# yeyupiaoling/PPASR

Hardware: AMD Instinct MI355X
Metric: audio-seconds/s (RTF^-1) Conformer-streaming fbank, batch32 per GPU, ctc_greedy (higher is better)
Workload: dtype f32

## Files before the change

### ppasr_amd/csrc/capi.hip

```cpp
#include <cxxabi.h>
#include <cstdlib>

#include "capi_internal.h"

namespace ppasr {
thread_local LaunchProf g_launch_prof;
}

static thread_local std::string g_err;
std::string& ppasr_err_slot() { return g_err; }


ppasr_status upload_pe_table(ppasr_model_s* m, BlobMap& sd, const float** pe_dev) {
  const int d = m->desc.output_size > 0 ? m->desc.output_size : kD;
  const int max_len = m->desc.max_len > 0 ? m->desc.max_len : 5000;
  m->desc.max_len = max_len;
  std::vector<float> pe((size_t)max_len * d);
  auto it = sd.find("__pe_table__");
  if (it != sd.end() && it->second.numel() == pe.size()) {
    std::memcpy(pe.data(), it->second.p, pe.size() * sizeof(float));
  } else {
    for (int i = 0; i < d / 2; ++i) {
      float div = expf((float)(2 * i) * (float)(-(std::log(10000.0) / d)));
      for (int pos = 0; pos < max_len; ++pos) {
// ... 152 lines not shown
    GET(istd, "encoder.global_cmvn.istd", F);
    GET(ew, "encoder.embed.out.0.weight", (size_t)F * d);
    GET(eb, "encoder.embed.out.0.bias", d);
    GET(lg, "encoder.embed.out.1.weight", d);
    GET(lb, "encoder.embed.out.1.bias", d);
    UP(vec_of(mean, F), m->front.cmvn_mean);
    UP(vec_of(istd, F), m->front.cmvn_istd);
    m->lin_kpad = (F + 255) / 256 * 256;
    UP4(pack_b(m->lin_kpad, d, [&](int k, int n) { return k < F ? ew[(size_t)k * d + n] : 0.f; }), m->front.embed_w);
    UP(vec_of(eb, d), m->front.embed_b);
    UP(vec_of(lg, d), m->lin_ln_g);
    UP(vec_of(lb, d), m->lin_ln_b);
    m->front.conv1_w = m->front.conv1_b = m->front.conv2_b = nullptr;
    m->front.conv2_w = nullptr;
  } else {
    GET(mean, "encoder.global_cmvn.mean", F);
    GET(istd, "encoder.global_cmvn.istd", F);
    GET(c1w, "encoder.embed.conv.0.weight", d * 9);
    GET(c1b, "encoder.embed.conv.0.bias", d);
    const int k2 = il == 6 ? 5 : 3;
    GET(c2w, "encoder.embed.conv.2.weight", (size_t)d * d * k2 * k2);
    GET(c2b, "encoder.embed.conv.2.bias", d);
    const std::string lin = il ? "encoder.embed.linear" : "encoder.embed.out.0";
    GET(ew, lin + ".weight", (size_t)d * F2 * d);
    GET(eb, lin + ".bias", d);
    UP(vec_of(mean, F), m->front.cmvn_mean);
    UP(vec_of(istd, F), m->front.cmvn_istd);
    std::vector<float> c1(9 * d);
    for (int c = 0; c < d; ++c)
      for (int j = 0; j < 9; ++j) c1[j * d + c] = c1w[c * 9 + j];
    UP(c1, m->front.conv1_w);
    UP(vec_of(c1b, d), m->front.conv1_b);
    const int taps2 = k2 * k2;
    UP4(pack_b(taps2 * d, d, [&](int k, int n) { return c2w[((size_t)n * d + (k % d)) * taps2 + (k / d)]; }), m->front.conv2_w);
    UP(vec_of(c2b, d), m->front.conv2_b);
    m->front.conv2_k = k2;
    m->front.conv2_s = il == 6 ? 3 : 2;
    m->front.conv3_w = nullptr;
    m->front.conv3_b = nullptr;
    if (il == 8) {
      GET(c3w, "encoder.embed.conv.4.weight", (size_t)d * d * 9);
      GET(c3b, "encoder.embed.conv.4.bias", d);
      UP4(pack_b(9 * d, d, [&](int k, int n) { return c3w[((size_t)n * d + (k % d)) * 9 + (k / d)]; }), m->front.conv3_w);
      UP(vec_of(c3b, d), m->front.conv3_b);
    }
    UP4(pack_b(F2 * d, d, [&](int k, int n) { return ew[((size_t)(k % d) * F2 + (k / d)) * d + n]; }), m->front.embed_w);
    UP(vec_of(eb, d), m->front.embed_b);
  }

  const float* pe_dev = nullptr;
  if ((st = upload_pe_table(m, sd, &pe_dev)) != PPASR_OK) return st;
  m->pe_dev = pe_dev;
  UP(std::vector<float>(d, 0.f), m->zero_vec);
  if (generic) m->gen_x.resize(desc->num_blocks);
  const int max_len = m->desc.max_len;
  m->layers.resize(desc->num_blocks);
  m->layer_ks.assign(desc->num_blocks, KS);
  m->layer_group.assign(desc->num_blocks, 1);
  for (int i = 0; i < desc->num_blocks; ++i) {
    LayerW& L = m->layers[i];
    const int KSi = eff ? (KS >> eff_strides_before(*desc, i)) : KS;
    const bool grouped = eff && ((desc->group_layer_mask >> i) & 1);
    m->layer_ks[i] = KSi;
    m->layer_group[i] = grouped ? desc->group_size : 1;
    const int pbn = grouped ? desc->group_size * d : d;
    const std::string p = "encoder.encoders." + std::to_string(i) + ".";
    auto ln = [&](const std::string& n, const float** g, const float** b) -> ppasr_status {
// ... 511 lines not shown
    };
    fn();
    g_launch_prof = LaunchProf{};
  };
  const bool eff = h->desc.model_type == PPASR_MODEL_EFFICIENT_CONFORMER;
  const bool skip = h->skip_padding && lens && !h->taps && h->desc.input_layer != 1;
  const bool skip_front = skip && h->desc.input_layer == 0;
  const int rc = h->desc.causal ? 0 : (h->desc.cnn_module_kernel - 1) / 2;
  const int slack_half = rc + 4, slack_full = eff ? 2 * slack_half + rc + 8 : rc + 4;
  auto pskip = [&](int Tcur, int mul_cur) {
    PadSkip ps;
    if (skip) {
      ps.lens = lens;
      ps.Tp = Tcur;
      ps.mul = mul_cur;
      ps.slack = mul_cur == sub ? slack_full : slack_half;
    }
    return ps;
  };
  const f32x4* conv2_h3 = h->gemm_mode == PPASR_GEMM_F16X3 ? h->conv2_w_h3 : nullptr;
  const bool conv12 = h->desc.input_layer == 0 && !conv2_h3 && conv12_enabled(h) && conv12_supported(h->front, F, F2);
  const PadSkip ps_front = skip_front ? pskip(Tp, sub) : PadSkip{};
  if (!conv12) timed(0, [&] { launch_conv1(feats, h->front, y1, B, T, F, T1, F1, st, ps_front); });
  if (h->desc.input_layer == 8) {
    timed(1, [&] {
      launch_conv_stage(y1, h->front.conv2_w, h->front.conv2_b, y2, B, T1, F1, fd.T2, F2, 3, 2, st);
      launch_conv_stage(y2, h->front.conv3_w, h->front.conv3_b, y1, B, fd.T2, F2, Tp, h->F3, 3, 2, st);
    });
    timed(2, [&] { launch_embed(y1, h->front, xa, M, h->F3 * kD, sqrtf((float)kD), false, st, PadSkip{}, ffn_split_for(h, M), y2); });
  } else {
    timed(1, [&] {
      int* tile_tab = (size_t)B + 2 <= ((size_t)M + 63) / 64 * 64 ? reinterpret_cast<int*>(ws + wl.rmax) : nullptr;
      if (conv12) launch_conv12(feats, h->front, y2, B, T, F, Tp, F2, st, ps_front, tile_tab);
      else launch_conv2(y1, h->front, y2, B, T1, F1, Tp, F2, st, ps_front, tile_tab, h->desc.input_layer == 0 ? conv2_h3 : nullptr);
    });
    timed(2, [&] {
      launch_embed(y2, h->front, xa, M, F2 * kD, sqrtf((float)kD), false, st, ps_front, wide_slices_for(h, M, F2), y1,
                   conv2_h3 ? h->embed_w_h3 : nullptr);
    });
  }
  tap(xa, (size_t)M * kD);
  const int n_chunks = h->desc.linear_units / 256;
  struct BlkTab { int Ti, R; int* tab; } btabs[4];
  int n_bt = 0;
  size_t bt_off = ((size_t)B + 2 + 15) / 16 * 16;
  const bool bt_ok = skip && block_tables_enabled() && (size_t)B + 2 <= ((size_t)M + 63) / 64 * 64;
  auto with_table = [&](PadSkip p, int Tcur, int R) {
    if (!bt_ok) return p;
    for (int k = 0; k < n_bt; ++k)
      if (btabs[k].Ti == Tcur && btabs[k].R == R) { p.tab = btabs[k].tab; return p; }
    const size_t n = 1 + ((size_t)B * Tcur + R - 1) / R;
    if (n_bt == 4 || bt_off + n > 2 * (((size_t)M + 63) / 64 * 64)) return p;
    int* t = reinterpret_cast<int*>(ws + wl.rmax) + bt_off;
    launch_block_table(p, B * Tcur, R, t, st);
    btabs[n_bt++] = BlkTab{Tcur, R, t};
    bt_off += (n + 15) / 16 * 16;
    p.tab = t;
    return p;
  };
  int Ti = Tp, mul = sub, pstride = 1;
  bool s1_done = false;
  for (int i = 0; i < h->desc.num_blocks; ++i) {
    const LayerW& L = h->layers[i];
    const int Mi = B * Ti;
    const int grp = h->layer_group[i];
    constexpr int fuse_min_blocks = 128;
// ... 757 lines not shown
```

### ppasr_amd/csrc/capi_internal.h

```cpp
#pragma once
#include <hip/hip_runtime.h>

#include <cmath>
#include <cstdio>
#include <cstring>
#include <memory>
#include <string>
#include <unordered_map>
#include <vector>

#include "../../include/ppasr_hip.h"
#include "conformer_kernels.h"
#include "launch.h"
#include "ctc_beam.h"

using namespace ppasr;

#include "squeezeformer_kernels.h"
#include "ds2_kernels.h"

std::string& ppasr_err_slot();
inline ppasr_status fail(ppasr_status s, const std::string& msg) {
  ppasr_err_slot() = msg;
  return s;
}
#define HIP_TRY(expr)                                                                              \
  do {                                                                                             \
    hipError_t _e = (expr);                                                                        \
    if (_e != hipSuccess) return fail(PPASR_EHIP, std::string(#expr) + ": " + hipGetErrorString(_e)); \
  } while (0)

struct Blob {
  const float* p;
  int ndim;
  int64_t shape[4];
  size_t numel() const {
    size_t n = 1;
    for (int i = 0; i < ndim; ++i) n *= (size_t)shape[i];
    return n;
  }
};

template <typename Acc>
inline std::vector<float> pack_b(int K, int N, Acc w) {
  const int n_tiles = (N + 31) / 32, G = K / 8;
  std::vector<float> out((size_t)n_tiles * G * 256, 0.f);
  for (int nt = 0; nt < n_tiles; ++nt)
    for (int g = 0; g < G; ++g)
      for (int l = 0; l < 64; ++l) {
        int n = nt * 32 + (l & 31);
        if (n >= N) continue;
        float* dst = &out[(((size_t)nt * G + g) * 64 + l) * 4];
        for (int j = 0; j < 4; ++j) dst[j] = w(8 * g + 4 * (l >> 5) + j, n);
      }
  return out;
}

typedef std::unordered_map<std::string, Blob> BlobMap;

inline unsigned eff_stride_mask(const ppasr_model_desc& d) {
  if (d.model_type != PPASR_MODEL_EFFICIENT_CONFORMER) return 0u;
  if (d.stride_layer_mask != 0) return (unsigned)d.stride_layer_mask;
  return d.stride_layer_idx >= 0 ? (1u << d.stride_layer_idx) : 0u;
}
inline int eff_strides_before(const ppasr_model_desc& d, int layer) {
  return __builtin_popcount(eff_stride_mask(d) & ((1u << layer) - 1u));
}

struct ppasr_model_s {
  ppasr_model_desc desc;
  int F1, F2;
  const f32x4* gen_head_w = nullptr;
  const float* gen_head_b = nullptr;
  int gen_vpad = 0;
  int F3 = 0;
  struct Front {
    int T1, T2, Tp;
  };
  int sub_rate() const { return desc.input_layer == 1 ? 1 : desc.input_layer ? desc.input_layer : 4; }
  int F_last() const { return desc.input_layer == 8 ? F3 : F2; }
  int min_frames() const { return desc.input_layer == 1 ? 1 : desc.input_layer == 6 ? 11 : desc.input_layer == 8 ? 15 : 7; }
  Front front_dims(int T) const {
    if (desc.input_layer == 1) return Front{0, 0, T};
    Front f{(T - 1) / 2, 0, 0};
    if (desc.input_layer == 6) {
      f.Tp = (f.T1 - 5) / 3 + 1;
    } else if (desc.input_layer == 8) {
      f.T2 = (f.T1 - 1) / 2;
// ... 151 lines not shown
```

### ppasr_amd/csrc/capi_squeezeformer.hip

```cpp
#include "capi_internal.h"

namespace {

struct Getter {
  BlobMap& sd;
  std::string missing;
  const float* operator()(const std::string& name, size_t numel) {
    auto it = sd.find(name);
    if (it == sd.end() || it->second.numel() != numel) {
      if (missing.empty()) missing = name;
      return nullptr;
    }
    return it->second.p;
  }
};

std::vector<float> vec_of(const float* p, size_t n) { return std::vector<float>(p, p + n); }

}

#define GETW(var, name, numel)                 \
  const float* var = get(name, (size_t)(numel)); \
  if (!var) return fail(PPASR_EMISSING, "missing or mis-shaped weight: " + get.missing)
#define UP(vec, dst) \
// ... 11 lines not shown
  ppasr_status st;
  const bool no_ada = (dsc.options & PPASR_OPT_SQ_NO_ADAPTIVE_SCALE) != 0;
  const std::vector<float> ones_d(d, 1.f), zeros_d(d, 0.f);
  auto adapt = [&](const float*& as, const float*& ab) {
    if (no_ada) {
      as = ones_d.data();
      ab = zeros_d.data();
    }
  };
  {
    GETW(mean, "encoder.global_cmvn.mean", F);
    GETW(istd, "encoder.global_cmvn.istd", F);
    GETW(c1w, "encoder.embed.pw_conv.weight", d * 9);
    GETW(c1b, "encoder.embed.pw_conv.bias", d);
    const float* c2w = get("encoder.embed.dw_conv.weight", (size_t)d * d * 9);
    const bool dw_stride = !c2w;
    if (!c2w) {
      get.missing.clear();
      c2w = get("encoder.embed.dw_conv.weight", (size_t)d * 9);
    }
    if (!c2w) return fail(PPASR_EMISSING, "missing or mis-shaped weight: " + get.missing);
    GETW(c2b, "encoder.embed.dw_conv.bias", d);
    GETW(ew, "encoder.embed.input_proj.0.weight", (size_t)d * F2 * d);
    GETW(eb, "encoder.embed.input_proj.0.bias", d);
    GETW(pg, "encoder.preln.weight", d);
    GETW(pb, "encoder.preln.bias", d);
    UP(vec_of(mean, F), m->front.cmvn_mean);
    UP(vec_of(istd, F), m->front.cmvn_istd);
    std::vector<float> c1(9 * d);
    for (int c = 0; c < d; ++c)
      for (int j = 0; j < 9; ++j) c1[j * d + c] = c1w[c * 9 + j];
    UP(c1, m->front.conv1_w);
    UP(vec_of(c1b, d), m->front.conv1_b);
    UP4(pack_b(9 * d, d, [&](int k, int n) {
          if (dw_stride) return (k % d) == n ? c2w[(size_t)n * 9 + (k / d)] : 0.f;
          return c2w[((size_t)n * d + (k % d)) * 9 + (k / d)];
        }), m->front.conv2_w);
    UP(vec_of(c2b, d), m->front.conv2_b);
    UP4(pack_b(F2 * d, d, [&](int k, int n) { return ew[((size_t)(k % d) * F2 + (k / d)) * d + n]; }), m->front.embed_w);
    UP(vec_of(eb, d), m->front.embed_b);
    UP(vec_of(pg, d), m->preln_g);
    UP(vec_of(pb, d), m->preln_b);
  }
  m->sq_layers.resize(L);
  for (int i = 0; i < L; ++i) {
    SqLayerW& W = m->sq_layers[i];
    const std::string p = "encoder.encoders." + std::to_string(i) + ".";
    auto ln = [&](const std::string& n, const float** g, const float** b) -> ppasr_status {
      const float* gw = get(p + n + ".weight", d);
      const float* gb = get(p + n + ".bias", d);
      if (!gw || !gb) return fail(PPASR_EMISSING, "missing or mis-shaped weight: " + get.missing);
      ppasr_status s1 = m->upload(vec_of(gw, d), g);
      return s1 != PPASR_OK ? s1 : m->upload(vec_of(gb, d), b);
    };
    if ((st = ln("layer_norm1", &W.ln1_g, &W.ln1_b)) != PPASR_OK) return st;
    if ((st = ln("layer_norm2", &W.ln2_g, &W.ln2_b)) != PPASR_OK) return st;
    if ((st = ln("layer_norm3", &W.ln3_g, &W.ln3_b)) != PPASR_OK) return st;
    if ((st = ln("layer_norm4", &W.ln4_g, &W.ln4_b)) != PPASR_OK) return st;
    W.cm_eps = 1e-5f;
    if (sd.find(p + "conv_module.norm._mean") != sd.end()) {
      const float* mean = get(p + "conv_module.norm._mean", d);
      const float* var = get(p + "conv_module.norm._variance", d);
      const float* gw = get(p + "conv_module.norm.weight", d);
      const float* gb = get(p + "conv_module.norm.bias", d);
      if (!mean || !var || !gw || !gb) return fail(PPASR_EMISSING, "missing or mis-shaped weight: " + get.missing);
      std::vector<float> sc(d), sh(d);
      for (int c = 0; c < d; ++c) {
        sc[c] = gw[c] / std::sqrt(var[c] + 1e-5f);
        sh[c] = gb[c] - mean[c] * sc[c];
      }
// ... 220 lines not shown
  const int rc = causal ? 0 : (KS - 1) / 2;
  auto pskip = [&](int Tcur, int mul_cur) {
    PadSkip ps;
    if (skip) {
      ps.lens = lens;
      ps.Tp = Tcur;
      ps.mul = mul_cur;
      ps.slack = mul_cur == 4 ? 2 * (rc + 4) + rc + 8 : rc + 4;
    }
    return ps;
  };
  const PadSkip psF = pskip(Tp, 4), psH = pskip(Tr, 8);
  int* tile_tab = (size_t)B + 2 <= ((size_t)M + 63) / 64 * 64 ? reinterpret_cast<int*>(ws + wl.rmax) : nullptr;
  const int rowsF = h->taps ? 32 : row_block_for(h, B, Tp, 4, psF.slack, skip);
  const int rowsH = h->taps ? 32 : row_block_for(h, B, Tr, 8, psH.slack, skip);
  PadSkip psF_rb = psF, psH_rb = psH;
  if (skip && tile_tab && block_tables_enabled()) {
    const int RF = rowsF == 16 ? 16 : 32, RH = rowsH == 16 ? 16 : 32;
    const size_t nF = 1 + ((size_t)M + RF - 1) / RF, nH = 1 + ((size_t)B * Tr + RH - 1) / RH;
    const size_t o1 = ((size_t)B + 2 + 15) / 16 * 16, o2 = o1 + (nF + 15) / 16 * 16;
    if (o2 + nH <= 2 * (((size_t)M + 63) / 64 * 64)) {
      int* base = reinterpret_cast<int*>(ws + wl.rmax);
      launch_block_table(psF, M, RF, base + o1, st);
      launch_block_table(psH, B * Tr, RH, base + o2, st);
      psF_rb.tab = base + o1;
      psH_rb.tab = base + o2;
    }
  }
  const f32x4* conv2_h3 = h->gemm_mode == PPASR_GEMM_F16X3 ? h->conv2_w_h3 : nullptr;
  if (!conv2_h3 && conv12_enabled(h) && conv12_supported(h->front, F, F2)) {
    launch_conv12(feats, h->front, y2, B, T, F, Tp, F2, st, psF, tile_tab);
  } else {
    launch_conv1(feats, h->front, y1, B, T, F, T1, F1, st, psF);
    launch_conv2(y1, h->front, y2, B, T1, F1, Tp, F2, st, psF, tile_tab, conv2_h3);
  }
  launch_embed(y2, h->front, xa, M, F2 * kD, sqrtf((float)kD), true, st,
               (rowsF != 16 && ffn_split_for(h, M) == 1) ? psF_rb : psF, ffn_split_for(h, M), y1,
               conv2_h3 ? h->embed_w_h3 : nullptr);
  launch_ln_rows(xa, h->preln_g, h->preln_b, M, st, psF);
  tap(xa, (size_t)M * kD);
  float* x = xa;
  float* other = xb;
  bool reduced = false;
  bool have_qkv = false;
  for (int i = 0; i < L; ++i) {
    const SqLayerW& W = h->sq_layers[i];
    if (i == h->desc.reduce_idx) {
      HIP_TRY(hipMemcpyAsync(xs, x, (size_t)M * kD * sizeof(float), hipMemcpyDeviceToDevice, st));
      launch_sq_reduce(x, other, qkv, h->sq_reduce, W.wqkv, W.bqkv, lens, B, Tp, Tr, st, psH);
      std::swap(x, other);
      reduced = true;
      have_qkv = true;
    }
    if (i == h->desc.recover_idx && reduced) {
      launch_sq_recover(x, xs, other, qkv, h->sq_wrec, h->sq_brec, W.wqkv, W.bqkv, B, Tp, Tr, st, psF);
      std::swap(x, other);
      reduced = false;
      have_qkv = true;
    }
    const int Ti = reduced ? Tr : Tp;
    const int Mi = B * Ti;
    const int mul = reduced ? 8 : 4;
    const PadSkip& ps = reduced ? psH : psF;
    const bool views16 = ffn_split_for(h, Mi) > 1 && !(rowsF == 16 && h->ffn_split < 0) && Mi <= kSplitRows16Max &&
                         !(h->gemm_mode == PPASR_GEMM_F16X3 && !h->sq_layers_h3.empty());
    auto qkv_view = [](const SqLayerW& w) {
      LayerW v{};
// ... 76 lines not shown
```

### ppasr_amd/csrc/conformer_kernels.h

```cpp
#pragma once
#include <hip/hip_runtime.h>
#include <stdint.h>

#include "rowblock.h"

namespace ppasr {

struct LayerW {
  const float *ln_mac_g, *ln_mac_b, *ln_mha_g, *ln_mha_b, *ln_conv_g, *ln_conv_b;
  const float *ln_ff_g, *ln_ff_b, *ln_fin_g, *ln_fin_b, *ln_cm_g, *ln_cm_b;
  float cm_eps;
  const f32x4 *ffm_w1, *ffm_w2, *ff_w1, *ff_w2, *wqkv, *wo, *pw1, *pw2;
  const float *ffm_b1, *ffm_b2, *ff_b1, *ff_b2, *bqkv, *bo, *pw1_b, *pw2_b;
  const float *dw_w;
  const float *dw_b;
  const float *glu_pad;
  const float *pos_u, *pos_v;
  const float *ptab;
};

struct FrontW {
  const float *cmvn_mean, *cmvn_istd;
  const float *conv1_w, *conv1_b;
  const f32x4 *conv2_w;
  const float *conv2_b;
  int conv2_k = 3, conv2_s = 2;
  const f32x4 *conv3_w = nullptr;
  const float *conv3_b = nullptr;
  const f32x4 *embed_w;
  const float *embed_b;
};

struct HeadW {
  const float *ln_g, *ln_b;
  const f32x4 *w;
  const float *b;
  int V, n_tiles;
};

struct SessDesc {
  int sess;
  int cache_t;
  int pos0;
  int pad;
};

struct AttnArgs {
  const float* q;
  int q_stride;
  const float* k;
  int k_stride;
  const float* v;
  int v_stride;
  int T1, T2;
  int pos0;
  const int64_t* lens;
  float* ctx;
  const float *pos_u, *pos_v;
  const float* ptab;
  int pos_stride;
  int mask_mul;
  int q_frames, kv_frames;
  int group;
  const SessDesc* sess;
  long long sess_stride;
  int pad_skip;
  const float* vt = nullptr;
  int vt_stride = 0;
  int dm = 256;
};
struct VtOut {
  float* vt = nullptr;
  int stride = 0;
  int k_h3 = 0;
};

constexpr size_t kLdsExclusive = 82 * 1024;
size_t ragged_lds(size_t lds, const PadSkip& ps, int n_blocks);

bool launch_attention_t(const AttnArgs& a, int B, int H, hipStream_t st);
hipError_t configure_attention_kernels();

void launch_block_table(const PadSkip& ps, int M, int R, int* tab, hipStream_t st);

bool conv12_supported(const FrontW& fw, int F, int F2);
void launch_conv12(const float* feats, const FrontW& fw, float* y2, int B, int T, int F, int Tp, int F2, hipStream_t st,
                   const PadSkip& ps_frames, int* tile_scratch);
hipError_t configure_front_fused_kernels();

void launch_ffn_qkv_16(const float* x_in, float* x1, float* qkv, const LayerW& w, int M, int n_chunks, hipStream_t st,
                       const PadSkip& ps);
void launch_out_glu_16(const float* ctx, const float* x1, float* x2, float* g, const LayerW& w, const int64_t* lens, int M,
                       int Tp, int mask_mul, hipStream_t st, const PadSkip& ps);
void launch_out_glu_split_16(const float* ctx, const float* x1, float* x2, float* g, float* xhat, const LayerW& w,
                             const int64_t* lens, int M, int Tp, int mask_mul, hipStream_t st, const PadSkip& ps,
                             float* hist = nullptr, int lo = 0);
void launch_shift_caches(float* kc, float* vc, long long layer_stride, int D, int n_layers, int from_full, int keep_full,
                         int from_half, int keep_half, unsigned long long half_mask, hipStream_t st);
void launch_oproj_ln_16(const float* ctx, const float* x1, float* x2_sink, float* xhat_out, const LayerW& w, int M,
                        hipStream_t st, const PadSkip& ps = PadSkip{});
void launch_pw1_glu_cols_16(const float* x, float* g, const LayerW& w, int M, hipStream_t st, float* hist = nullptr, int lo = 0,
                            const float* hist_scale = nullptr, const float* hist_bias = nullptr, const PadSkip& ps = PadSkip{},
                            const int64_t* lens = nullptr, int Tp = 1, int mask_mul = 1);
bool conv_ffn_16_supported(int ksize, int Tp);
void launch_conv_ffn_16(const float* g, const float* x2, float* x_out, const LayerW& w, const int64_t* lens, int M, int Tp,
                        int n_chunks, int ksize, int mask_mul, const LayerW* next, float* x1_next, float* qkv_next,
                        hipStream_t st, bool causal, const PadSkip& ps);
void launch_ffn_qkv_w16(const float* x_in, float* x1, float* qkv, const LayerW& w, int M, int n_chunks, hipStream_t st,
                        const PadSkip& ps, VtOut vt);
void launch_out_glu_w16(const float* ctx, const float* x1, float* x2, float* g, const LayerW& w, const int64_t* lens, int M,
                        int Tp, int mask_mul, hipStream_t st, const PadSkip& ps);
void launch_conv_ffn_w16(const float* g, const float* x2, float* x_out, const LayerW& w, const int64_t* lens, int M, int Tp,
                         int n_chunks, int ksize, int mask_mul, const LayerW* next, float* x1_next, float* qkv_next,
                         hipStream_t st, bool causal, const PadSkip& ps, VtOut vt_next);
hipError_t configure_conformer_t_kernels();

void launch_posproj(const float* pe, const float* wpos , const float* bpos_or_null, float* ptab,
                    int max_len, hipStream_t st, int d = 256);
void launch_conv1(const float* feats, const FrontW& fw, float* y1, int B, int T, int F, int T1, int F1, hipStream_t st,
                  const PadSkip& ps = PadSkip{}, int channels = 256);
// ... 107 lines not shown
```

### ppasr_amd/csrc/front_fused.hip

```cpp
#include "conformer_kernels.h"
#include "launch.h"

namespace ppasr {

template <int MT>
__global__ __launch_bounds__(kThreads) void k_conv12(const float* __restrict__ feats, FrontW fw, float* __restrict__ out,
                                                     int T, int F, int Tp, int F2, int M, int m0, PadSkip ps,
                                                     const int* __restrict__ tile_tab) {
  constexpr int BM = 32 * MT, KC = 128, LD = KC + 4, G = KC / 8, NL = 2 * MT, STEP = G / NL, N_CHUNKS = 18;
  int r0 = m0 + blockIdx.x * BM, Mlim = M;
  if (tile_tab) {
    const int t = blockIdx.x, nb = tile_tab[0];
    const int* pre = tile_tab + 1;
    if (t >= pre[nb]) return;
    int lo = 0, hi = nb;
    while (hi - lo > 1) {
      const int mid = (lo + hi) >> 1;
      if (pre[mid] <= t) lo = mid;
      else hi = mid;
    }
    const int S = ps.Tp * ps.unit;
    r0 = lo * S + (t - pre[lo]) * BM;
    Mlim = min(M, (lo + 1) * S);
  } else if (pad_block_skippable(ps, r0, BM, M)) {
    return;
  }
  extern __shared__ __attribute__((aligned(16))) float smem[];
  float* xs = smem + 2 * BM * LD;
  const int tid = threadIdx.x, lane = lane_id(), wave = wave_id();
  constexpr int tile_stride = N_CHUNKS * G * 64;
  const f32x4* wbase = fw.conv2_w + (size_t)wave * tile_stride;
  BRing<1> ring;
  ring_prime(ring, wbase, 0);
  const int bt0 = r0 / F2, nbt = (min(r0 + BM, Mlim) - 1) / F2 - bt0 + 1;
  for (int idx = tid; idx < nbt * 7 * F; idx += kThreads) {
    const int p = idx / F, f = idx - p * F;
    const int btl = p / 7, fr = p - 7 * btl;
    const int bt = bt0 + btl, b = bt / Tp, tp = bt - b * Tp;
    const int t = min(4 * tp + fr, T - 1);
    xs[idx] = (feats[((size_t)b * T + t) * F + f] - fw.cmvn_mean[f]) * fw.cmvn_istd[f];
  }
  const int c4 = tid & 31, rbase = tid >> 5;
  uint32_t pb[MT];
#pragma unroll
  for (int i = 0; i < NL; ++i) {
    const int m = r0 + rbase + 16 * i;
    const int bt = m / F2, f2 = m - bt * F2;
    const uint32_t v = m < Mlim ? (uint32_t)((bt - bt0) * 7 * F + 4 * f2) : 0xffffu;
    pb[i >> 1] = (i & 1) ? (pb[i >> 1] | (v << 16)) : v;
  }
  auto pbase = [&](int i) { return (int)((i & 1) ? (pb[i >> 1] >> 16) : (pb[i >> 1] & 0xffffu)); };
  const int lds_off0 = rbase * LD + 4 * c4;
  f32x4 wv[9], bv;
  float xv[9];
  auto load_w = [&](int kc) {
    const int c = (kc & 1) * 128 + 4 * c4;
#pragma unroll
    for (int j = 0; j < 9; ++j) wv[j] = *reinterpret_cast<const f32x4*>(fw.conv1_w + j * 256 + c);
    bv = *reinterpret_cast<const f32x4*>(fw.conv1_b + c);
  };
  auto read_x = [&](int i, int toff) {
    const int o = pbase(i);
    const float* p = xs + (o == 0xffff ? 0 : o) + toff;
#pragma unroll
    for (int ii = 0; ii < 3; ++ii)
#pragma unroll
      for (int jj = 0; jj < 3; ++jj) xv[ii * 3 + jj] = p[ii * F + jj];
  };
  auto fma_row = [&](int i, float* buf) {
    f32x4 a = {0.f, 0.f, 0.f, 0.f};
#pragma unroll
    for (int j = 0; j < 9; ++j)
#pragma unroll
      for (int e = 0; e < 4; ++e) a[e] = fmaf(wv[j][e], xv[j], a[e]);
    a += bv;
#pragma unroll
    for (int e = 0; e < 4; ++e) a[e] = pbase(i) != 0xffff ? fmaxf(a[e], 0.f) : 0.f;
    *reinterpret_cast<f32x4*>(buf + lds_off0 + i * 16 * LD) = a;
  };
  auto tap_off = [&](int kc) {
    const int tap = kc >> 1, kh = tap / 3, kw = tap - 3 * kh;
    return 2 * kh * F + 2 * kw;
  };
  f32x16 acc[MT][1];
  acc_zero(acc);
  load_w(0);
  __syncthreads();
#pragma unroll
  for (int i = 0; i < NL; ++i) {
    read_x(i, 0);
    fma_row(i, smem);
  }
  __syncthreads();
  for (int kc = 0; kc < N_CHUNKS; ++kc) {
    float* cur = smem + (kc & 1) * BM * LD;
    float* nxt = smem + ((kc + 1) & 1) * BM * LD;
    const f32x4* seg = wbase + (size_t)kc * G * 64;
    if (kc + 1 < N_CHUNKS) {
      load_w(kc + 1);
      const int toff = tap_off(kc + 1);
      auto side = [&](int g) {
        const int i = g / STEP, ph = g - i * STEP;
        if (i < NL && ph == 0) read_x(i, toff);
        if (i < NL && ph == 1) fma_row(i, nxt);
      };
      rb_gemm<MT, 1, G, kPF, decltype(side)>(cur, LD, seg, 0, seg + G * 64, 0, ring, acc, side);
    } else {
      rb_gemm<MT, 1, G>(cur, LD, seg, 0, nullptr, 0, ring, acc);
    }
    __syncthreads();
  }
  const int col = wave * 32 + (lane & 31);
  const float b2 = fw.conv2_b[col];
#pragma unroll
  for (int mt = 0; mt < MT; ++mt)
#pragma unroll
    for (int r = 0; r < 16; ++r) {
      const int m = r0 + mt * 32 + acc_row(r, lane);
      const float v = fmaxf((acc[mt][0][r] + b2) * 1.0f, 0.f);
      if (m < Mlim) out[(size_t)m * 256 + col] = v;
    }
}

static size_t conv12_lds(int mt, int F, int F2) {
  const int bm = 32 * mt, nbt = (bm - 1) / F2 + 2;
  return ((size_t)2 * bm * 132 + (size_t)nbt * 7 * F) * sizeof(float);
}
bool conv12_supported(const FrontW& fw, int F, int F2) {
  return fw.conv2_k == 3 && fw.conv2_s == 2 && F2 >= 1 && conv12_lds(4, F, F2) <= 160 * 1024 &&
         (size_t)((127 / F2) + 2) * 7 * F < 0xffff;
}

void launch_tile_prefix(const PadSkip& ps, int B, int BM, int* tab, hipStream_t st);

void launch_conv12(const float* feats, const FrontW& fw, float* y2, int B, int T, int F, int Tp, int F2, hipStream_t st,
                   const PadSkip& ps_frames, int* tile_scratch) {
  PadSkip ps = ps_frames;
  ps.unit = F2;
  const int M = B * Tp * F2;
  constexpr int kCUs = 256;
  const int* no_tab = nullptr;
#define CONV12(MTA, GRID, M0, TAB)                                                                                      \
  PPASR_LAUNCH(k_conv12<MTA>, dim3(GRID), dim3(kThreads), conv12_lds(MTA, F, F2), st, feats, fw, y2, T, F, Tp, F2, M, M0, \
               ps, TAB)
  if (ps.lens && tile_scratch && M > 128 * kCUs) {
    launch_tile_prefix(ps, B, 128, tile_scratch, st);
    const int per_utt = (Tp * F2 + 127) / 128;
    CONV12(4, B * per_utt, 0, (const int*)tile_scratch);
    return;
  }
  const int tiles4 = (M + 127) / 128;
  const int full = (tiles4 / kCUs) * kCUs;
  const int rem_rows = M - full * 128;
  const int mt_rem = (rem_rows + 32 * kCUs - 1) / (32 * kCUs);
  if (full == 0) {
    const int mt = (M + 32 * kCUs - 1) / (32 * kCUs);
    if (mt <= 1) CONV12(1, (M + 31) / 32, 0, no_tab);
    else if (mt == 2) CONV12(2, (M + 63) / 64, 0, no_tab);
    else if (mt == 3) CONV12(3, (M + 95) / 96, 0, no_tab);
    else CONV12(4, (M + 127) / 128, 0, no_tab);
    return;
  }
  if (rem_rows <= 0 || mt_rem >= 4) {
    CONV12(4, tiles4, 0, no_tab);
    return;
  }
  CONV12(4, full, 0, no_tab);
  const int m0 = full * 128;
  if (mt_rem <= 1) CONV12(1, (rem_rows + 31) / 32, m0, no_tab);
  else if (mt_rem == 2) CONV12(2, (rem_rows + 63) / 64, m0, no_tab);
  else CONV12(3, (rem_rows + 95) / 96, m0, no_tab);
#undef CONV12
}

hipError_t configure_front_fused_kernels() {
  hipError_t e;
#define SET_LDS(fn)                                                                                              \
  e = hipFuncSetAttribute(reinterpret_cast<const void*>(fn), hipFuncAttributeMaxDynamicSharedMemorySize, 160 * 1024); \
  if (e != hipSuccess) return e;
  SET_LDS(k_conv12<1>);
  SET_LDS(k_conv12<2>);
  SET_LDS(k_conv12<3>);
  SET_LDS(k_conv12<4>);
#undef SET_LDS
  return hipSuccess;
}

}
```

Baseline: 54250.

## Compute conv2 output time-pairs with shared-tap Winograd-style F(2,3) decomposition

Rewrites the subsampling conv2 (3x3, stride 2) so each block computes two adjacent output time steps together. Along the time axis it uses a Winograd-like 1D F(2,3) split: it forms differences of input rows (d0-d1, d2-d1) and combines weights (g0, w1, g0+g1, g1), packed on the host into a new conv2_wp layout. The goal is fewer GEMM k-chunks per output and shared y1 loads across the pair. It also adds a standalone pair kernel for the unfused y1 path and always launches MT=1 tiles instead of the CU-aware MT mix, which may lower per-block reuse and change occupancy. Summing pre-combined weights also slightly changes f32 rounding.

```diff
diff --git a/ppasr_amd/csrc/capi.hip b/ppasr_amd/csrc/capi.hip
--- a/ppasr_amd/csrc/capi.hip
+++ b/ppasr_amd/csrc/capi.hip
@@ -208,7 +208,10 @@
     UP(c1, m->front.conv1_w);
     UP(vec_of(c1b, d), m->front.conv1_b);
     const int taps2 = k2 * k2;
-    UP4(pack_b(taps2 * d, d, [&](int k, int n) { return c2w[((size_t)n * d + (k % d)) * taps2 + (k / d)]; }), m->front.conv2_w);
+    auto c2 = [&](int k, int n) { return c2w[((size_t)n * d + (k % d)) * taps2 + (k / d)]; };
+    UP4(pack_b(taps2 * d, d, c2), m->front.conv2_w);
+    m->front.conv2_wp = nullptr;
+    if (il == 0 && d == kD) UP4(pack_conv2_pair(d, c2), m->front.conv2_wp);
     UP(vec_of(c2b, d), m->front.conv2_b);
     m->front.conv2_k = k2;
     m->front.conv2_s = il == 6 ? 3 : 2;
@@ -786,6 +789,8 @@
     timed(1, [&] {
       int* tile_tab = (size_t)B + 2 <= ((size_t)M + 63) / 64 * 64 ? reinterpret_cast<int*>(ws + wl.rmax) : nullptr;
       if (conv12) launch_conv12(feats, h->front, y2, B, T, F, Tp, F2, st, ps_front, tile_tab);
+      else if (h->desc.input_layer == 0 && !conv2_h3 && conv2_pair_supported(h->front))
+        launch_conv2_pair(y1, h->front, y2, B, T1, F1, Tp, F2, st, ps_front, tile_tab);
       else launch_conv2(y1, h->front, y2, B, T1, F1, Tp, F2, st, ps_front, tile_tab, h->desc.input_layer == 0 ? conv2_h3 : nullptr);
     });
     timed(2, [&] {
diff --git a/ppasr_amd/csrc/capi_internal.h b/ppasr_amd/csrc/capi_internal.h
--- a/ppasr_amd/csrc/capi_internal.h
+++ b/ppasr_amd/csrc/capi_internal.h
@@ -54,6 +54,15 @@
         for (int j = 0; j < 4; ++j) dst[j] = w(8 * g + 4 * (l >> 5) + j, n);
       }
   return out;
+}
+
+template <typename Acc>
+inline std::vector<float> pack_conv2_pair(int d, Acc w) {
+  return pack_b(24 * 128, d, [&](int k, int n) {
+    const int s = k / 512, slab = (k / 128) & 3, kw = s >> 1, c = (s & 1) * 128 + (k & 127);
+    const float g0 = w(kw * d + c, n), w1 = w((3 + kw) * d + c, n), g1 = w((6 + kw) * d + c, n);
+    return slab == 0 ? g0 : slab == 1 ? w1 : slab == 2 ? g0 + g1 : g1;
+  });
 }
 
 typedef std::unordered_map<std::string, Blob> BlobMap;
diff --git a/ppasr_amd/csrc/capi_squeezeformer.hip b/ppasr_amd/csrc/capi_squeezeformer.hip
--- a/ppasr_amd/csrc/capi_squeezeformer.hip
+++ b/ppasr_amd/csrc/capi_squeezeformer.hip
@@ -67,10 +67,12 @@
       for (int j = 0; j < 9; ++j) c1[j * d + c] = c1w[c * 9 + j];
     UP(c1, m->front.conv1_w);
     UP(vec_of(c1b, d), m->front.conv1_b);
-    UP4(pack_b(9 * d, d, [&](int k, int n) {
-          if (dw_stride) return (k % d) == n ? c2w[(size_t)n * 9 + (k / d)] : 0.f;
-          return c2w[((size_t)n * d + (k % d)) * 9 + (k / d)];
-        }), m->front.conv2_w);
+    auto c2 = [&](int k, int n) {
+      if (dw_stride) return (k % d) == n ? c2w[(size_t)n * 9 + (k / d)] : 0.f;
+      return c2w[((size_t)n * d + (k % d)) * 9 + (k / d)];
+    };
+    UP4(pack_b(9 * d, d, c2), m->front.conv2_w);
+    if (d == kD) UP4(pack_conv2_pair(d, c2), m->front.conv2_wp);
     UP(vec_of(c2b, d), m->front.conv2_b);
     UP4(pack_b(F2 * d, d, [&](int k, int n) { return ew[((size_t)(k % d) * F2 + (k / d)) * d + n]; }), m->front.embed_w);
     UP(vec_of(eb, d), m->front.embed_b);
@@ -357,7 +359,8 @@
     launch_conv12(feats, h->front, y2, B, T, F, Tp, F2, st, psF, tile_tab);
   } else {
     launch_conv1(feats, h->front, y1, B, T, F, T1, F1, st, psF);
-    launch_conv2(y1, h->front, y2, B, T1, F1, Tp, F2, st, psF, tile_tab, conv2_h3);
+    if (!conv2_h3 && conv2_pair_supported(h->front)) launch_conv2_pair(y1, h->front, y2, B, T1, F1, Tp, F2, st, psF, tile_tab);
+    else launch_conv2(y1, h->front, y2, B, T1, F1, Tp, F2, st, psF, tile_tab, conv2_h3);
   }
   launch_embed(y2, h->front, xa, M, F2 * kD, sqrtf((float)kD), true, st,
                (rowsF != 16 && ffn_split_for(h, M) == 1) ? psF_rb : psF, ffn_split_for(h, M), y1,
diff --git a/ppasr_amd/csrc/conformer_kernels.h b/ppasr_amd/csrc/conformer_kernels.h
--- a/ppasr_amd/csrc/conformer_kernels.h
+++ b/ppasr_amd/csrc/conformer_kernels.h
@@ -23,6 +23,7 @@
   const float *cmvn_mean, *cmvn_istd;
   const float *conv1_w, *conv1_b;
   const f32x4 *conv2_w;
+  const f32x4 *conv2_wp = nullptr;
   const float *conv2_b;
   int conv2_k = 3, conv2_s = 2;
   const f32x4 *conv3_w = nullptr;
@@ -83,9 +84,12 @@
 
 void launch_block_table(const PadSkip& ps, int M, int R, int* tab, hipStream_t st);
 
+bool conv2_pair_supported(const FrontW& fw);
 bool conv12_supported(const FrontW& fw, int F, int F2);
 void launch_conv12(const float* feats, const FrontW& fw, float* y2, int B, int T, int F, int Tp, int F2, hipStream_t st,
                    const PadSkip& ps_frames, int* tile_scratch);
+void launch_conv2_pair(const float* y1, const FrontW& fw, float* y2, int B, int T1, int F1, int Tp, int F2, hipStream_t st,
+                       const PadSkip& ps_frames, int* tile_scratch);
 hipError_t configure_front_fused_kernels();
 
 void launch_ffn_qkv_16(const float* x_in, float* x1, float* qkv, const LayerW& w, int M, int n_chunks, hipStream_t st,
diff --git a/ppasr_amd/csrc/front_fused.hip b/ppasr_amd/csrc/front_fused.hip
--- a/ppasr_amd/csrc/front_fused.hip
+++ b/ppasr_amd/csrc/front_fused.hip
@@ -3,12 +3,14 @@
 
 namespace ppasr {
 
-template <int MT>
-__global__ __launch_bounds__(kThreads) void k_conv12(const float* __restrict__ feats, FrontW fw, float* __restrict__ out,
-                                                     int T, int F, int Tp, int F2, int M, int m0, PadSkip ps,
-                                                     const int* __restrict__ tile_tab) {
-  constexpr int BM = 32 * MT, KC = 128, LD = KC + 4, G = KC / 8, NL = 2 * MT, STEP = G / NL, N_CHUNKS = 18;
-  int r0 = m0 + blockIdx.x * BM, Mlim = M;
+template <int MT, bool FROM_Y1>
+__device__ __forceinline__ void conv2_pair_body(const float* __restrict__ src, const FrontW& fw, float* __restrict__ out,
+                                                int T, int F, int Tp, int F2, int M, int m0, const PadSkip& ps,
+                                                const int* __restrict__ tile_tab) {
+  constexpr int BP = 32 * MT, KC = 128, LD = KC + 4, G = KC / 8, NL = 2 * MT, N_STAGES = 6, N_CHUNKS = 4 * N_STAGES;
+  constexpr int SLOT = 2 * BP * LD;
+  const int P = (Tp + 1) >> 1;
+  int r0 = m0 + blockIdx.x * BP, Mlim = M;
   if (tile_tab) {
     const int t = blockIdx.x, nb = tile_tab[0];
     const int* pre = tile_tab + 1;
@@ -20,93 +22,160 @@
       else hi = mid;
     }
     const int S = ps.Tp * ps.unit;
-    r0 = lo * S + (t - pre[lo]) * BM;
+    r0 = lo * S + (t - pre[lo]) * BP;
     Mlim = min(M, (lo + 1) * S);
-  } else if (pad_block_skippable(ps, r0, BM, M)) {
+  } else if (pad_block_skippable(ps, r0, BP, M)) {
     return;
   }
   extern __shared__ __attribute__((aligned(16))) float smem[];
-  float* xs = smem + 2 * BM * LD;
+  float* const slot0 = smem;
+  float* const slot1 = smem + SLOT;
   const int tid = threadIdx.x, lane = lane_id(), wave = wave_id();
   constexpr int tile_stride = N_CHUNKS * G * 64;
-  const f32x4* wbase = fw.conv2_w + (size_t)wave * tile_stride;
+  const f32x4* wbase = fw.conv2_wp + (size_t)wave * tile_stride;
   BRing<1> ring;
   ring_prime(ring, wbase, 0);
-  const int bt0 = r0 / F2, nbt = (min(r0 + BM, Mlim) - 1) / F2 - bt0 + 1;
-  for (int idx = tid; idx < nbt * 7 * F; idx += kThreads) {
-    const int p = idx / F, f = idx - p * F;
-    const int btl = p / 7, fr = p - 7 * btl;
-    const int bt = bt0 + btl, b = bt / Tp, tp = bt - b * Tp;
-    const int t = min(4 * tp + fr, T - 1);
-    xs[idx] = (feats[((size_t)b * T + t) * F + f] - fw.cmvn_mean[f]) * fw.cmvn_istd[f];
-  }
   const int c4 = tid & 31, rbase = tid >> 5;
+  const int bp0 = r0 / F2;
+  float* xs = smem + 2 * SLOT;
   uint32_t pb[MT];
-#pragma unroll
-  for (int i = 0; i < NL; ++i) {
-    const int m = r0 + rbase + 16 * i;
-    const int bt = m / F2, f2 = m - bt * F2;
-    const uint32_t v = m < Mlim ? (uint32_t)((bt - bt0) * 7 * F + 4 * f2) : 0xffffu;
-    pb[i >> 1] = (i & 1) ? (pb[i >> 1] | (v << 16)) : v;
+  int yrow[FROM_Y1 ? NL : 1], yp4[FROM_Y1 ? NL : 1], yf[FROM_Y1 ? NL : 1];
+  if constexpr (!FROM_Y1) {
+    const int nbp = (min(r0 + BP, Mlim) - 1) / F2 - bp0 + 1;
+    for (int idx = tid; idx < nbp * 11 * F; idx += kThreads) {
+      const int q = idx / F, f = idx - q * F;
+      const int bpl = q / 11, fr = q - 11 * bpl;
+      const int bp = bp0 + bpl, b = bp / P, p = bp - b * P;
+      const int t = min(8 * p + fr, T - 1);
+      xs[idx] = (src[((size_t)b * T + t) * F + f] - fw.cmvn_mean[f]) * fw.cmvn_istd[f];
+    }
+#pragma unroll
+    for (int i = 0; i < NL; ++i) {
+      const int m = r0 + rbase + 16 * i;
+      const int bp = m / F2, f2 = m - bp * F2;
+      const uint32_t v = m < Mlim ? (uint32_t)((bp - bp0) * 11 * F + 4 * f2) : 0xffffu;
+      pb[i >> 1] = (i & 1) ? (pb[i >> 1] | (v << 16)) : v;
+    }
+  } else {
+#pragma unroll
+    for (int i = 0; i < NL; ++i) {
+      const int m = r0 + rbase + 16 * i;
+      const int bp = m / F2, f2 = m - bp * F2, b = bp / P, p = bp - b * P;
+      yrow[i] = b * T + 4 * p;
+      yp4[i] = 4 * p;
+      yf[i] = m < Mlim ? 2 * f2 : -1;
+    }
   }
   auto pbase = [&](int i) { return (int)((i & 1) ? (pb[i >> 1] >> 16) : (pb[i >> 1] & 0xffffu)); };
   const int lds_off0 = rbase * LD + 4 * c4;
-  f32x4 wv[9], bv;
+  f32x4 wv[FROM_Y1 ? 1 : 9], bv;
   float xv[9];
-  auto load_w = [&](int kc) {
-    const int c = (kc & 1) * 128 + 4 * c4;
-#pragma unroll
-    for (int j = 0; j < 9; ++j) wv[j] = *reinterpret_cast<const f32x4*>(fw.conv1_w + j * 256 + c);
-    bv = *reinterpret_cast<const f32x4*>(fw.conv1_b + c);
-  };
-  auto read_x = [&](int i, int toff) {
-    const int o = pbase(i);
-    const float* p = xs + (o == 0xffff ? 0 : o) + toff;
-#pragma unroll
-    for (int ii = 0; ii < 3; ++ii)
-#pragma unroll
-      for (int jj = 0; jj < 3; ++jj) xv[ii * 3 + jj] = p[ii * F + jj];
-  };
-  auto fma_row = [&](int i, float* buf) {
-    f32x4 a = {0.f, 0.f, 0.f, 0.f};
-#pragma unroll
-    for (int j = 0; j < 9; ++j)
-#pragma unroll
-      for (int e = 0; e < 4; ++e) a[e] = fmaf(wv[j][e], xv[j], a[e]);
-    a += bv;
-#pragma unroll
-    for (int e = 0; e < 4; ++e) a[e] = pbase(i) != 0xffff ? fmaxf(a[e], 0.f) : 0.f;
-    *reinterpret_cast<f32x4*>(buf + lds_off0 + i * 16 * LD) = a;
-  };
-  auto tap_off = [&](int kc) {
-    const int tap = kc >> 1, kh = tap / 3, kw = tap - 3 * kh;
-    return 2 * kh * F + 2 * kw;
-  };
-  f32x16 acc[MT][1];
-  acc_zero(acc);
+  f32x4 yv;
+  auto load_w = [&](int s) {
+    if constexpr (!FROM_Y1) {
+      const int c = (s & 1) * 128 + 4 * c4;
+#pragma unroll
+      for (int j = 0; j < 9; ++j) wv[j] = *reinterpret_cast<const f32x4*>(fw.conv1_w + j * 256 + c);
+      bv = *reinterpret_cast<const f32x4*>(fw.conv1_b + c);
+    }
+  };
+  auto y1_read = [&](int i, int s, int j) {
+    const int kw = s >> 1;
+    if constexpr (!FROM_Y1) {
+      const int o = pbase(i);
+      const float* p = xs + (o == 0xffff ? 0 : o) + 2 * j * F + 2 * kw;
+#pragma unroll
+      for (int ii = 0; ii < 3; ++ii)
+#pragma unroll
+        for (int jj = 0; jj < 3; ++jj) xv[ii * 3 + jj] = p[ii * F + jj];
+    } else {
+      yv = f32x4{0.f, 0.f, 0.f, 0.f};
+      if (yf[i] >= 0 && yp4[i] + j < T)
+        yv = *reinterpret_cast<const f32x4*>(src + ((size_t)(yrow[i] + j) * F + yf[i] + kw) * 256 + (s & 1) * 128 + 4 * c4);
+    }
+  };
+  auto y1_value = [&](int i) {
+    if constexpr (!FROM_Y1) {
+      f32x4 a = {0.f, 0.f, 0.f, 0.f};
+#pragma unroll
+      for (int j = 0; j < 9; ++j)
+#pragma unroll
+        for (int e = 0; e < 4; ++e) a[e] = fmaf(wv[j][e], xv[j], a[e]);
+      a += bv;
+#pragma unroll
+      for (int e = 0; e < 4; ++e) a[e] = pbase(i) != 0xffff ? fmaxf(a[e], 0.f) : 0.f;
+      return a;
+    } else {
+      return yv;
+    }
+  };
+  auto put = [&](float* buf, int row16, const f32x4& v) {
+    *reinterpret_cast<f32x4*>(buf + lds_off0 + row16 * 16 * LD) = v;
+  };
+  f32x4 d1c[NL], d0;
+  auto side_d01 = [&](int s, int g) {
+    const int e = g >> 1, i = e >> 1;
+    if (e >= 2 * NL) return;
+    if ((g & 1) == 0) {
+      y1_read(i, s, (e & 1) ? 2 : 0);
+    } else if ((e & 1) == 0) {
+      d0 = y1_value(i);
+    } else {
+      d1c[i] = y1_value(i);
+      put(slot0, i, d0 - d1c[i]);
+    }
+  };
+  auto side_o = [&](int s, int g) {
+    const int e = g >> 1, hi = e >= NL, i = e - (hi ? NL : 0);
+    if (e >= 2 * NL) return;
+    if ((g & 1) == 0) y1_read(i, s, hi ? 3 : 1);
+    else put(slot1, hi ? NL + i : i, y1_value(i));
+  };
+  auto side_d1 = [&](int g) {
+    if (g < NL) put(slot0, g, d1c[g]);
+  };
+  auto side_d21 = [&](int s, int g) {
+    const int e = g >> 1;
+    if (e >= NL) return;
+    if ((g & 1) == 0) y1_read(e, s, 4);
+    else put(slot1, e, y1_value(e) - d1c[e]);
+  };
   load_w(0);
   __syncthreads();
 #pragma unroll
-  for (int i = 0; i < NL; ++i) {
-    read_x(i, 0);
-    fma_row(i, smem);
+  for (int g = 0; g < 2 * G; ++g) {
+    side_d01(0, g);
+    __builtin_amdgcn_sched_barrier(0);
   }
   __syncthreads();
-  for (int kc = 0; kc < N_CHUNKS; ++kc) {
-    float* cur = smem + (kc & 1) * BM * LD;
-    float* nxt = smem + ((kc + 1) & 1) * BM * LD;
-    const f32x4* seg = wbase + (size_t)kc * G * 64;
-    if (kc + 1 < N_CHUNKS) {
-      load_w(kc + 1);
-      const int toff = tap_off(kc + 1);
-      auto side = [&](int g) {
-        const int i = g / STEP, ph = g - i * STEP;
-        if (i < NL && ph == 0) read_x(i, toff);
-        if (i < NL && ph == 1) fma_row(i, nxt);
-      };
-      rb_gemm<MT, 1, G, kPF, decltype(side)>(cur, LD, seg, 0, seg + G * 64, 0, ring, acc, side);
-    } else {
-      rb_gemm<MT, 1, G>(cur, LD, seg, 0, nullptr, 0, ring, acc);
+  f32x16 accA[MT][1], accB[MT][1], accS[MT][1];
+  acc_zero(accA);
+  acc_zero(accB);
+  acc_zero(accS);
+  for (int s = 0; s < N_STAGES; ++s) {
+    const f32x4* seg = wbase + (size_t)(4 * s) * G * 64;
+    {
+      auto side = [&](int g) { side_o(s, g); };
+      rb_gemm<MT, 1, G, kPF, decltype(side)>(slot0, LD, seg, 0, seg + G * 64, 0, ring, accA, side);
+    }
+    __syncthreads();
+    {
+      auto side = [&](int g) { side_d1(g); };
+      rb_gemm<MT, 1, G, kPF, decltype(side)>(slot1, LD, seg + G * 64, 0, seg + G * 64, 0, ring, accA, side);
+      rb_gemm<MT, 1, G>(slot1 + BP * LD, LD, seg + G * 64, 0, seg + 2 * G * 64, 0, ring, accB);
+    }
+    __syncthreads();
+    {
+      auto side = [&](int g) { side_d21(s, g); };
+      rb_gemm<MT, 1, G, kPF, decltype(side)>(slot0, LD, seg + 2 * G * 64, 0, seg + 3 * G * 64, 0, ring, accS, side);
+    }
+    __syncthreads();
+    if (s + 1 < N_STAGES) {
+      load_w(s + 1);
+      auto side = [&](int g) { side_d01(s + 1, g); };
+      rb_gemm<MT, 1, G, kPF, decltype(side)>(slot1, LD, seg + 3 * G * 64, 0, seg + 4 * G * 64, 0, ring, accB, side);
+    } else {
+      rb_gemm<MT, 1, G>(slot1, LD, seg + 3 * G * 64, 0, nullptr, 0, ring, accB);
     }
     __syncthreads();
   }
@@ -117,60 +186,75 @@
 #pragma unroll
     for (int r = 0; r < 16; ++r) {
       const int m = r0 + mt * 32 + acc_row(r, lane);
-      const float v = fmaxf((acc[mt][0][r] + b2) * 1.0f, 0.f);
-      if (m < Mlim) out[(size_t)m * 256 + col] = v;
-    }
-}
-
-static size_t conv12_lds(int mt, int F, int F2) {
-  const int bm = 32 * mt, nbt = (bm - 1) / F2 + 2;
-  return ((size_t)2 * bm * 132 + (size_t)nbt * 7 * F) * sizeof(float);
-}
+      if (m >= Mlim) continue;
+      const int bp = m / F2, f2 = m - bp * F2, b = bp / P, t0 = 2 * (bp - b * P);
+      const float s = accS[mt][0][r];
+      float* o = out + ((size_t)(b * Tp + t0) * F2 + f2) * 256 + col;
+      o[0] = fmaxf(accA[mt][0][r] + s + b2, 0.f);
+      if (t0 + 1 < Tp) o[(size_t)F2 * 256] = fmaxf(s + accB[mt][0][r] + b2, 0.f);
+    }
+}
+
+template <int MT>
+__global__ __launch_bounds__(kThreads) void k_conv12(const float* __restrict__ feats, FrontW fw, float* __restrict__ out,
+                                                     int T, int F, int Tp, int F2, int M, int m0, PadSkip ps,
+                                                     const int* __restrict__ tile_tab) {
+  conv2_pair_body<MT, false>(feats, fw, out, T, F, Tp, F2, M, m0, ps, tile_tab);
+}
+template <int MT>
+__global__ __launch_bounds__(kThreads) void k_conv2_pair(const float* __restrict__ y1, FrontW fw, float* __restrict__ out,
+                                                         int T1, int F1, int Tp, int F2, int M, int m0, PadSkip ps,
+                                                         const int* __restrict__ tile_tab) {
+  conv2_pair_body<MT, true>(y1, fw, out, T1, F1, Tp, F2, M, m0, ps, tile_tab);
+}
+
+static size_t pair_lds(int mt, bool fused, int F, int F2) {
+  const int bp = 32 * mt, nbp = (bp - 1) / F2 + 2;
+  return ((size_t)2 * 2 * bp * 132 + (fused ? (size_t)nbp * 11 * F : 0)) * sizeof(float);
+}
+bool conv2_pair_supported(const FrontW& fw) { return fw.conv2_wp && fw.conv2_k == 3 && fw.conv2_s == 2; }
 bool conv12_supported(const FrontW& fw, int F, int F2) {
-  return fw.conv2_k == 3 && fw.conv2_s == 2 && F2 >= 1 && conv12_lds(4, F, F2) <= 160 * 1024 &&
-         (size_t)((127 / F2) + 2) * 7 * F < 0xffff;
+  return conv2_pair_supported(fw) && F2 >= 1 && pair_lds(1, true, F, F2) <= 160 * 1024 &&
+         (size_t)((31 / F2) + 2) * 11 * F < 0xffff;
 }
 
 void launch_tile_prefix(const PadSkip& ps, int B, int BM, int* tab, hipStream_t st);
+
+static void launch_pair(bool fused, const float* src, const FrontW& fw, float* y2, int B, int T, int F, int Tp, int F2,
+                        hipStream_t st, const PadSkip& ps_frames, int* tile_scratch) {
+  const int P = (Tp + 1) / 2;
+  PadSkip ps = ps_frames;
+  ps.Tp = P;
+  ps.mul = 2 * ps_frames.mul;
+  ps.slack = (ps_frames.slack + 1) / 2;
+  ps.unit = F2;
+  const int M = B * P * F2;
+  const int* no_tab = nullptr;
+#define PAIR(MTA, GRID, M0, TAB)                                                                                        \
+  do {                                                                                                                 \
+    if (fused)                                                                                                         \
+      PPASR_LAUNCH(k_conv12<MTA>, dim3(GRID), dim3(kThreads), pair_lds(MTA, true, F, F2), st, src, fw, y2, T, F, Tp, F2, \
+                   M, M0, ps, TAB);                                                                                    \
+    else                                                                                                               \
+      PPASR_LAUNCH(k_conv2_pair<MTA>, dim3(GRID), dim3(kThreads), pair_lds(MTA, false, F, F2), st, src, fw, y2, T, F,   \
+                   Tp, F2, M, M0, ps, TAB);                                                                            \
+  } while (0)
+  if (ps.lens && tile_scratch) {
+    launch_tile_prefix(ps, B, 32, tile_scratch, st);
+    PAIR(1, B * ((P * F2 + 31) / 32), 0, (const int*)tile_scratch);
+    return;
+  }
+  PAIR(1, (M + 31) / 32, 0, no_tab);
+#undef PAIR
+}
 
 void launch_conv12(const float* feats, const FrontW& fw, float* y2, int B, int T, int F, int Tp, int F2, hipStream_t st,
                    const PadSkip& ps_frames, int* tile_scratch) {
-  PadSkip ps = ps_frames;
-  ps.unit = F2;
-  const int M = B * Tp * F2;
-  constexpr int kCUs = 256;
-  const int* no_tab = nullptr;
-#define CONV12(MTA, GRID, M0, TAB)                                                                                      \
-  PPASR_LAUNCH(k_conv12<MTA>, dim3(GRID), dim3(kThreads), conv12_lds(MTA, F, F2), st, feats, fw, y2, T, F, Tp, F2, M, M0, \
-               ps, TAB)
-  if (ps.lens && tile_scratch && M > 128 * kCUs) {
-    launch_tile_prefix(ps, B, 128, tile_scratch, st);
-    const int per_utt = (Tp * F2 + 127) / 128;
-    CONV12(4, B * per_utt, 0, (const int*)tile_scratch);
-    return;
-  }
-  const int tiles4 = (M + 127) / 128;
-  const int full = (tiles4 / kCUs) * kCUs;
-  const int rem_rows = M - full * 128;
-  const int mt_rem = (rem_rows + 32 * kCUs - 1) / (32 * kCUs);
-  if (full == 0) {
-    const int mt = (M + 32 * kCUs - 1) / (32 * kCUs);
-    if (mt <= 1) CONV12(1, (M + 31) / 32, 0, no_tab);
-    else if (mt == 2) CONV12(2, (M + 63) / 64, 0, no_tab);
-    else if (mt == 3) CONV12(3, (M + 95) / 96, 0, no_tab);
-    else CONV12(4, (M + 127) / 128, 0, no_tab);
-    return;
-  }
-  if (rem_rows <= 0 || mt_rem >= 4) {
-    CONV12(4, tiles4, 0, no_tab);
-    return;
-  }
-  CONV12(4, full, 0, no_tab);
-  const int m0 = full * 128;
-  if (mt_rem <= 1) CONV12(1, (rem_rows + 31) / 32, m0, no_tab);
-  else if (mt_rem == 2) CONV12(2, (rem_rows + 63) / 64, m0, no_tab);
-  else CONV12(3, (rem_rows + 95) / 96, m0, no_tab);
-#undef CONV12
+  launch_pair(true, feats, fw, y2, B, T, F, Tp, F2, st, ps_frames, tile_scratch);
+}
+void launch_conv2_pair(const float* y1, const FrontW& fw, float* y2, int B, int T1, int F1, int Tp, int F2, hipStream_t st,
+                       const PadSkip& ps_frames, int* tile_scratch) {
+  launch_pair(false, y1, fw, y2, B, T1, F1, Tp, F2, st, ps_frames, tile_scratch);
 }
 
 hipError_t configure_front_fused_kernels() {
@@ -179,9 +263,7 @@
   e = hipFuncSetAttribute(reinterpret_cast<const void*>(fn), hipFuncAttributeMaxDynamicSharedMemorySize, 160 * 1024); \
   if (e != hipSuccess) return e;
   SET_LDS(k_conv12<1>);
-  SET_LDS(k_conv12<2>);
-  SET_LDS(k_conv12<3>);
-  SET_LDS(k_conv12<4>);
+  SET_LDS(k_conv2_pair<1>);
 #undef SET_LDS
   return hipSuccess;
 }
```

Result: faster. 55770, median of 6 (+2.8%).
